# int-brain-lab/mtscomp

Hardware: AMD Instinct MI355X
Metric: compress + decompress GB/s (raw int16) (higher is better)
Workload: dtype int16

## Files before the change

### mtscomp_amd/csrc/inflate.hip

```cpp
#include <stdlib.h>

#include <vector>

#include "common.h"

namespace mts {

struct BitIn {
    const u32 *w;
    u64 nwords;
    u64 widx;
    u64 buf;
    u32 cnt;
    u32 nextw;
    u64 pos;
    u64 end;
    const u32 *lw = nullptr;
    u64 lw0 = 0;
    u32 lwn = 0;
    __device__ __forceinline__ void init(const u8 *base, u64 byte_off, u64 byte_len, u64 start_bit)
    {
        const u64 a = (u64)(base + byte_off);
        w = (const u32 *)(a & ~(u64)3);
        const u64 bit0 = (a & 3) * 8;
// ... 1624 lines not shown
            u32 x = valid ? nt : 0, y = valid ? no : 0;
#pragma unroll
            for (int off = 1; off < 64; off <<= 1) {
                const u32 xx = __shfl_up(x, off, 64), yy = __shfl_up(y, off, 64);
                if (lane >= off) { x += xx; y += yy; }
            }
            __syncthreads();
            if (lane == 63) { s_wt[wave] = x; s_wo[wave] = y; }
            __syncthreads();
            u32 pre_t = 0, pre_o = 0, rt = 0, ro = 0;
#pragma unroll
            for (int w = 0; w < WV_NT / 64; w++) { const u32 a = s_wt[w], bb = s_wo[w]; if (w < wave) { pre_t += a; pre_o += bb; } rt += a; ro += bb; }
            if (nout + ro > limit) emit = false;
            bool bad = false;
            if (valid) {
                u32 *out = tk + ntok + pre_t + (x - nt);
                u64 have = nout + pre_o + (y - no);
                bl.seek(start);
                u32 k = 0;
                while (k < nt) {
                    u32 tok, olen;
                    if (decode_token_lut(bl, L, lutl, lutd, tok, olen) != 0) { bad = true; break; }
                    if ((tok >> 31) && (u64)((tok & 0x7fff) + 1) > have) { bad = true; break; }
                    if (emit) lz_emit_pieces(out + k, tok, olen);
                    k += lz_pieces(tok, olen); have += olen;
                }
            }
            if (tid == 0) s_any = 0;
            __syncthreads();
            if (__any(bad) && lane == 0) s_any = 1;
            if (fstop < WV_NT && tid == fstop) { s_wstop[0] = (u32)fl; s_wstop[1] = ex; }
            if (fstop == WV_NT && tid == WV_NT - 1) s_wstop[1] = ex;
            __syncthreads();
            if (s_any) { st = INF_CORRUPT; break; }
            ntok += emit ? rt : 0; nout += ro;
            if (fstop < WV_NT) {
                if ((int)s_wstop[0] == SPAN_EOB) { done = true; pos = (wb0 << 5) + s_wstop[1]; }
                else st = INF_CORRUPT;
            } else base = (wb0 << 5) + s_wstop[1];
        }
    }
    if (st != INF_OK) r.status = MTS_CHUNK_CORRUPT;
    else {
        const u64 tb = (pos + 7) & ~7ull;
        if (tb + 32 > br.end) r.status = MTS_CHUNK_CORRUPT;
        else {
            const u8 *t = (const u8 *)br.w + (tb >> 3);
            r.adler_stored = ((u32)t[0] << 24) | ((u32)t[1] << 16) | ((u32)t[2] << 8) | t[3];
            r.end_bit = tb + 32;
            if (!emit || nout != limit) r.status = MTS_CHUNK_BADSIZE;
        }
    }
    r.n_out = (u32)(nout < 0xffffffffull ? nout : 0xffffffffull); r.ntok = ntok;
    if (tid == 0) res[ci] = r;
}

constexpr int LZ_THREADS = 1024;
constexpr int LZ_FLUSHERS = 2;
constexpr int LZ_WORKERS = LZ_THREADS / 64 - LZ_FLUSHERS;
constexpr u32 LZ_RING = 65536;
constexpr u32 LZ_REACH = 32768 + 258;
constexpr u32 LZ_FLUSH = 4096;
constexpr u32 LZ_ZLAG = 10;
constexpr u32 LZ_AHEAD = LZ_RING - LZ_ZLAG * LZ_FLUSH;
static_assert(LZ_REACH <= (LZ_ZLAG - 1) * LZ_FLUSH, "a slot must be out of every copy's reach before it is zeroed");
constexpr u32 LZ_BITS_OFF = LZ_RING;
constexpr u32 LZ_CTL_OFF = LZ_RING + LZ_RING / 8 + 16;
constexpr int LZ_LDS = LZ_CTL_OFF + 256;
constexpr u32 LZ_EDGE = LZ_RING - 12;
constexpr u32 LZ_SPIN_MAX = 1u << 20;

#ifndef MTS_LZ_MAXSEG
#define MTS_LZ_MAXSEG 32
#endif
constexpr int LZ_MAXSEG = MTS_LZ_MAXSEG;
constexpr int LZ_STATUS_RETRY = 1000;
constexpr u32 LZ_WIN = 32768;
struct LzPlan {
    u32 nseg;
    u32 g0[LZ_MAXSEG + 1];
    u32 b0[LZ_MAXSEG + 1];
};
constexpr u32 LZ2_CTL_OFF = 2 * LZ_RING + 16;
constexpr int LZ2_LDS = LZ2_CTL_OFF + 256;

constexpr int GS_TILE = 256;

__global__ __launch_bounds__(GS_TILE) void k_inf_gsum(const u32 *__restrict__ tokens, const InfChunk *__restrict__ chunks,
                                                      const InfResult *__restrict__ res, const u64 *__restrict__ gb_off,
                                                      const u64 *__restrict__ tb_off, u32 *__restrict__ gbase,
                                                      u32 *__restrict__ tile_base)
{
    const int ci = blockIdx.y;
    const InfResult r = res[ci];
    if (r.status != MTS_CHUNK_OK) return;
    const u32 ntok = r.ntok, ngroups = (ntok + 63) / 64;
    const u32 g = blockIdx.x * GS_TILE + threadIdx.x;
    if (blockIdx.x * GS_TILE >= ngroups && !(blockIdx.x == 0)) return;
    const u32 *tk = tokens + chunks[ci].tok_off;
    u32 sum = 0;
    {
        const int lane_ = threadIdx.x & 63;
        const u32 g0w = g - (u32)lane_;
        const uint4 *q = (const uint4 *)(tk + (size_t)g0w * 64);
        const u32 nq = ntok > g0w * 64 ? (ntok - g0w * 64) / 4 : 0;
#pragma unroll
        for (int it = 0; it < 16; it++) {
            const u32 i = (u32)it * 64 + (u32)lane_;
            u32 part = 0;
            if (i < nq) {
                const uint4 v = q[i];
                part = ((v.x >> 31) ? ((v.x >> 16) & 0xff) + 3 : 1) + ((v.y >> 31) ? ((v.y >> 16) & 0xff) + 3 : 1) +
                       ((v.z >> 31) ? ((v.z >> 16) & 0xff) + 3 : 1) + ((v.w >> 31) ? ((v.w >> 16) & 0xff) + 3 : 1);
            }
            part += (u32)__builtin_amdgcn_update_dpp(0, (int)part, 0x111, 0xf, 0xf, false);
            part += (u32)__builtin_amdgcn_update_dpp(0, (int)part, 0x112, 0xf, 0xf, false);
            part += (u32)__builtin_amdgcn_update_dpp(0, (int)part, 0x114, 0xf, 0xf, false);
            part += (u32)__builtin_amdgcn_update_dpp(0, (int)part, 0x118, 0xf, 0xf, false);
            const u32 got = (u32)__shfl((int)part, (lane_ & 3) * 16 + 15, 64);
            if ((lane_ >> 2) == it) sum = got;
        }
        if (g < ngroups) {
            const u32 t0 = g * 64, t1 = min(t0 + 64, ntok);
            for (u32 i = max(t0, (g0w * 64 + nq * 4)); i < t1; i++) { const u32 t = tk[i]; sum += (t >> 31) ? ((t >> 16) & 0xff) + 3 : 1; }
        } else sum = 0;
    }
    __shared__ u32 wtot[GS_TILE / 64];
    const int wave = threadIdx.x >> 6, lane = threadIdx.x & 63;
    u32 x = sum;
#pragma unroll
    for (int off = 1; off < 64; off <<= 1) { const u32 y = __shfl_up(x, off, 64); if (lane >= off) x += y; }
    if (lane == 63) wtot[wave] = x;
    __syncthreads();
    u32 add = 0, tot = 0;
    for (int w = 0; w < GS_TILE / 64; w++) { if (w < wave) add += wtot[w]; tot += wtot[w]; }
    if (g < ngroups) gbase[gb_off[ci] + g] = add + x - sum;
    if (threadIdx.x == 0) tile_base[tb_off[ci] + blockIdx.x] = tot;
}

__global__ __launch_bounds__(64) void k_inf_gscan(const InfResult *__restrict__ res, const u64 *__restrict__ tb_off,
                                                  u32 *__restrict__ tile_base)
{
    const int ci = blockIdx.x;
    const InfResult r = res[ci];
    if (r.status != MTS_CHUNK_OK) return;
    const u32 ngroups = (r.ntok + 63) / 64, ntiles = (ngroups + GS_TILE - 1) / GS_TILE;
    u32 *tb = tile_base + tb_off[ci];
    const int lane = threadIdx.x;
    u32 carry = 0;
    for (u32 t0 = 0; t0 < ntiles; t0 += 64) {
        const u32 v = t0 + lane < ntiles ? tb[t0 + lane] : 0;
        u32 x = v;
#pragma unroll
        for (int off = 1; off < 64; off <<= 1) { const u32 y = __shfl_up(x, off, 64); if (lane >= off) x += y; }
        if (t0 + lane < ntiles) tb[t0 + lane] = carry + x - v;
        carry += __shfl(x, 63, 64);
    }
}

__device__ __forceinline__ u32 wave_incl_scan_dpp(u32 x)
{
    x += (u32)__builtin_amdgcn_update_dpp(0, (int)x, 0x111, 0xf, 0xf, false);
    x += (u32)__builtin_amdgcn_update_dpp(0, (int)x, 0x112, 0xf, 0xf, false);
    x += (u32)__builtin_amdgcn_update_dpp(0, (int)x, 0x114, 0xf, 0xf, false);
    x += (u32)__builtin_amdgcn_update_dpp(0, (int)x, 0x118, 0xf, 0xf, false);
    x += (u32)__builtin_amdgcn_update_dpp(0, (int)x, 0x142, 0xa, 0xf, false);
    x += (u32)__builtin_amdgcn_update_dpp(0, (int)x, 0x143, 0xc, 0xf, false);
// ... 205 lines not shown
            }
            const u64 pn = ballot64(pv != 0);
            u64 nx = pn;
            if (pn != pm || (pn & slowm)) idle = 0;
            else if (__builtin_amdgcn_readfirstlane((int)lds_ld(lds_bad))) nx = 0;
            else if (++idle > (1u << 22)) { nx = 0; lds_st(lds_bad, 2); }
            else __builtin_amdgcn_s_sleep(4);
            pm = nx;
        }
        if (prof) { const u64 c3_ = __builtin_readcyclecounter(); pc_wait += c1_ - c0_; pc_pre += c2_ - c1_; pc_loop += c3_ - c2_; pc_groups++; }
    }
    if (prof && lane == 0) {
        u64 *q = prof + ((u64)ci * 16 + wave) * 8;
        q[0] = __builtin_readcyclecounter() - pc_t0; q[1] = pc_wait; q[2] = pc_pre; q[3] = pc_loop; q[4] = pc_iter; q[5] = pc_groups; q[6] = pc_vm; q[7] = pc_sleeps;
    }
    if (lane == 0) lds_st(lds_prog + 4 * wave, 0xffffffffu);
    if (wave == 0) {
        for (u32 waits = 0; flushed() < nout && waits < 4 * LZ_SPIN_MAX; waits++) __builtin_amdgcn_s_sleep(8);
        if (lane == 0 && (lds_ld(lds_bad) || flushed() < nout)) res[ci].status = (pass || lds_ld(lds_bad) == 1) ? MTS_CHUNK_CORRUPT : LZ_STATUS_RETRY;
    }
}

__device__ __forceinline__ void lz2_load_window(u32 data_addr, u32 &x0, u32 &x1, u32 &x2, u32 &x3, u32 &x4)
{
    u32x2 p, q;
    asm volatile("ds_read2_b32 %0, %3 offset1:1\n\tds_read2_b32 %1, %3 offset0:2 offset1:3\n\t"
                 "ds_read_b32 %2, %3 offset:16\n\ts_waitcnt lgkmcnt(0)"
                 : "=&v"(p), "=&v"(q), "=&v"(x4) : "v"(data_addr) : "memory");
    x0 = p.x; x1 = p.y; x2 = q.x; x3 = q.y;
}
__device__ __forceinline__ void lz2_or_window(u32 data_addr, u32 o0, u32 o1, u32 o2, u32 o3, u32 o4)
{
    asm volatile("ds_or_b32 %0, %1\n\tds_or_b32 %0, %2 offset:4\n\tds_or_b32 %0, %3 offset:8\n\tds_or_b32 %0, %4 offset:12\n\t"
                 "ds_or_b32 %0, %5 offset:16"
                 :: "v"(data_addr), "v"(o0), "v"(o1), "v"(o2), "v"(o3), "v"(o4) : "memory");
}
__device__ __forceinline__ void lz2_or_cell(u32 data_addr, u32 w) { asm volatile("ds_or_b32 %0, %1" :: "v"(data_addr), "v"(w) : "memory"); }
__device__ __forceinline__ u32 lz2_load_cell(u32 data_addr)
{
    u32 data;
    asm volatile("ds_read_u16 %0, %1\n\ts_waitcnt lgkmcnt(0)" : "=&v"(data) : "v"(data_addr) : "memory");
    return data;
}
__device__ __forceinline__ u32 lz2_zero_half(u32 y) { return (y - 0x00010001u) & ~y & 0x80008000u; }
__device__ __forceinline__ u32 lz2_pk_min(u32 a, u32 b) { u32 d; asm("v_pk_min_u16 %0, %1, %2" : "=v"(d) : "v"(a), "v"(b)); return d; }

__global__ __launch_bounds__(64) void k_inf_plan(const InfResult *__restrict__ res, const u64 *__restrict__ gb_off,
                                                 const u64 *__restrict__ tb_off, const u32 *__restrict__ gbase,
                                                 const u32 *__restrict__ tile_base, int n_chunks, int nseg_req, LzPlan *__restrict__ plan)
{
    const int ci = blockIdx.x * 64 + threadIdx.x;
    if (ci >= n_chunks) return;
    const InfResult r = res[ci];
    LzPlan *p = plan + ci;
    p->nseg = 1;
    for (int k = 0; k <= LZ_MAXSEG; k++) { p->g0[k] = 0; p->b0[k] = 0; }
    if (r.status == MTS_CHUNK_OK && r.ntok) {
        const u32 ngroups = (r.ntok + 63) / 64;
        const u32 *gbl = gbase + gb_off[ci];
        const u32 *tbs = tile_base + tb_off[ci];
        auto gb = [&](u32 g) -> u32 { return g >= ngroups ? r.n_out : tbs[g / GS_TILE] + gbl[g]; };
        p->g0[1] = ngroups; p->b0[1] = r.n_out;
        for (int ns = nseg_req; ns > 1; ns >>= 1) {
            const u32 per = (ngroups + ns - 1) / ns;
            bool ok = per > 0;
            u32 prev_g = 0, prev_b = 0;
            for (int k = 1; k <= ns && ok; k++) {
                const u32 g = min((u32)k * per, ngroups), b = gb(g);
                if (g <= prev_g) ok = false;
                if (k < ns && b - prev_b < LZ_WIN + 512) ok = false;
                prev_g = g; prev_b = b;
            }
            if (!ok) continue;
            p->nseg = (u32)ns;
            for (int k = 0; k <= ns; k++) { const u32 g = min((u32)k * per, ngroups); p->g0[k] = g; p->b0[k] = gb(g); }
            break;
        }
    }
}
#ifndef MTS_LZ2_STATS
#define MTS_LZ2_STATS 0
#endif
#if MTS_LZ2_STATS
__device__ unsigned long long g_lz2_stats[16];
#define LZ2_CLK() __builtin_readcyclecounter()
#endif
__global__ __launch_bounds__(LZ_THREADS) void k_inf_lz_seg(const u32 *__restrict__ tokens, const InfChunk *__restrict__ chunks,
                                                           InfResult *__restrict__ res, const u64 *__restrict__ gb_off,
                                                           const u64 *__restrict__ tb_off, const u32 *__restrict__ gbase,
                                                           const u32 *__restrict__ tile_base, const LzPlan *__restrict__ plan,
                                                           u16 *__restrict__ sym, int n_workers, int pass, u8 *__restrict__ stream,
                                                           u8 *__restrict__ gflag, u64 *__restrict__ seg_adler)
{
    const int ci = blockIdx.y, seg = blockIdx.x;
    const InfResult r = res[ci];
    if (pass == 2) { if (threadIdx.x == 0 && seg == 0 && r.status == MTS_CHUNK_OK && plan[ci].nseg >= 2) res[ci].status = LZ_STATUS_RETRY; return; }
    if (r.status != (pass ? LZ_STATUS_RETRY : MTS_CHUNK_OK)) return;
    const LzPlan *pl = plan + ci;
    if (pl->nseg < 2 || (u32)seg >= pl->nseg) return;
    const InfChunk ch = chunks[ci];
    extern __shared__ __attribute__((aligned(16))) u8 smem[];
    const u32 lds_data = (u32)(uintptr_t)smem;
    const u32 lds_prog = lds_data + LZ2_CTL_OFF;
    const u32 lds_flnext = lds_prog + 64;
    const u32 lds_bad = lds_prog + 80;
    const int wave = __builtin_amdgcn_readfirstlane((int)(threadIdx.x >> 6)), lane = threadIdx.x & 63;
    const u32 *tk = tokens + ch.tok_off;
    const u32 *gbl = gbase + gb_off[ci];
    const u32 *tbs = tile_base + tb_off[ci];
    u16 *out = sym + ch.stream_off;
    const u32 ntok = r.ntok, ngroups = (ntok + 63) / 64;
    const u32 g_lo = pl->g0[seg], g_hi = pl->g0[seg + 1], B = pl->b0[seg], Bend = pl->b0[seg + 1];
    for (u32 i = threadIdx.x * 16; i < LZ2_CTL_OFF; i += LZ_THREADS * 16) lds_zero16(lds_data + i);
    const u32 q0 = B / LZ_FLUSH;
    if (threadIdx.x < 24) {
        u32 v = 0;
        if (threadIdx.x >= 16 && threadIdx.x < 16 + LZ_FLUSHERS) { const u32 k = threadIdx.x - 16; v = (q0 + ((k - q0) & (LZ_FLUSHERS - 1))) * LZ_FLUSH; }
        lds_st(lds_prog + 4 * threadIdx.x, v);
    }
    __syncthreads();
    if (seg > 0) {
        for (u32 i = threadIdx.x; i < LZ_WIN; i += LZ_THREADS) {
            const u32 ro = (B - LZ_WIN + i) & (LZ_RING - 1);
            lz2_or_cell(lds_data + ((2 * ro) & ~3u), (256 + i + 1) << (16 * (ro & 1)));
        }
    }
    u32 t_n = 0, tb0_n = 0, gl0_n = 0, tb1_n = 0, gl1_n = 0;
    const int LZW = n_workers;
    auto prefetch = [&](u32 h) {
        const u32 h0 = h < g_hi ? h : g_hi - 1, h1 = h + 1 < ngroups ? h + 1 : ngroups - 1;
        const u32 i2 = h0 * 64 + lane;
        t_n = tk[i2 < ntok ? i2 : ntok - 1];
        tb0_n = tbs[h0 / GS_TILE]; gl0_n = gbl[h0]; tb1_n = tbs[h1 / GS_TILE]; gl1_n = gbl[h1];
    };
    if (wave < LZW) {
        prefetch(g_lo + wave);
        if (lane == 0) lds_st(lds_prog + 4 * wave, g_lo + (u32)wave < g_hi ? tb0_n + gl0_n : 0xffffffffu);
    }
    __syncthreads();
    auto safe_bytes = [&]() -> u32 {
        const u32 v = row0_min_dpp(lane < LZW ? lds_ld(lds_prog + 4 * lane) : 0xffffffffu);
        return v < Bend ? v : Bend;
    };
    auto flushed = [&]() -> u32 {
        u32 v = lds_ld(lds_flnext);
#pragma unroll
        for (int k = 1; k < LZ_FLUSHERS; k++) v = min(v, lds_ld(lds_flnext + 4 * k));
        return v;
    };
    if (wave >= LZ_WORKERS) {
        const u32 me = wave - LZ_WORKERS;
        u32 idle = 0;
        u8 *bytes_out = stream + ch.stream_off;
        u8 *gf = gflag + (ch.stream_off >> 12) + ci;
        const u64 nn = ch.n_expect;
        u64 sa = 0, sb = 0;
        for (u32 q = q0 + ((me - q0) & (LZ_FLUSHERS - 1));; q += LZ_FLUSHERS) {
            const u32 lo = q * LZ_FLUSH;
            if (lo >= Bend) break;
            const u32 hi = lo + LZ_FLUSH < Bend ? lo + LZ_FLUSH : Bend;
            while (safe_bytes() < hi) {
                if (++idle > LZ_SPIN_MAX || lds_ld(lds_bad)) { if (lane == 0) { if (!lds_ld(lds_bad)) lds_st(lds_bad, 3); for (int k = 0; k < LZ_FLUSHERS; k++) lds_st(lds_flnext + 4 * k, 0xffffffffu); } return; }
                __builtin_amdgcn_s_sleep(2);
            }
            idle = 0;
            const bool whole = lo >= B && hi == lo + LZ_FLUSH;
            u32x4 c[LZ_FLUSH / 512];
            u32 high = 0;
#pragma unroll
            for (u32 st = 0; st < LZ_FLUSH / 512; st++) {
                const u32 o = lo + st * 512 + lane * 8;
                c[st] = u32x4{0, 0, 0, 0};
                if (o < hi && o + 8 > B) asm volatile("ds_read_b128 %0, %1\n\ts_waitcnt lgkmcnt(0)" : "=v"(c[st]) : "v"(lds_data + 2 * (o & (LZ_RING - 1))) : "memory");
                if (whole || (o >= B && o + 8 <= hi)) { c[st].x -= 0x00010001u; c[st].y -= 0x00010001u; c[st].z -= 0x00010001u; c[st].w -= 0x00010001u; }
                high |= c[st].x | c[st].y | c[st].z | c[st].w;
            }
            if (whole && !any64((high & 0xff00ff00u) != 0)) {
#pragma unroll
                for (u32 st = 0; st < LZ_FLUSH / 512; st++) {
                    const u32 o = lo + st * 512 + lane * 8;
                    const u32 cw[4] = {c[st].x, c[st].y, c[st].z, c[st].w};
                    u32 d[2] = {0, 0}, s1 = 0, s2 = 0;
#pragma unroll
                    for (u32 k = 0; k < 8; k++) {
                        const u32 v = (cw[k >> 1] >> (16 * (k & 1))) & 0xff;
                        d[k >> 2] |= v << (8 * (k & 3));
                        s1 += v; s2 += k * v;
                    }
                    *(uint2 *)(bytes_out + o) = make_uint2(d[0], d[1]);
                    sa += s1; sb += (nn - o) * (u64)s1 - s2;
                }
            } else {
                if (lane == 0) gf[q] = 1;
#pragma unroll
                for (u32 st = 0; st < LZ_FLUSH / 512; st++) {
                    const u32 o = lo + st * 512 + lane * 8;
                    if (o < hi && o + 8 > B) {
                        if (o >= B && o + 8 <= hi) *(u32x4 *)(out + o) = c[st];
                        else { const u32 cw[4] = {c[st].x, c[st].y, c[st].z, c[st].w}; for (u32 k = 0; k < 8; k++) if (o + k >= B && o + k < hi) out[o + k] = (u16)((cw[k >> 1] >> (16 * (k & 1))) - 1u); }
                    }
                }
            }
            if (q >= LZ_ZLAG) {
                const u32 zo = ((q - LZ_ZLAG) * LZ_FLUSH) & (LZ_RING - 1);
#pragma unroll
                for (u32 o = lane * 16; o < 2 * LZ_FLUSH; o += 1024) lds_zero16(lds_data + 2 * zo + o);
            }
            if (lane == 0) lds_st(lds_flnext + 4 * me, lo + LZ_FLUSHERS * LZ_FLUSH);
        }
        for (int d = 32; d; d >>= 1) {
            sa += ((u64)(u32)__shfl_xor((u32)(sa >> 32), d) << 32) | (u32)__shfl_xor((u32)sa, d);
            sb += ((u64)(u32)__shfl_xor((u32)(sb >> 32), d) << 32) | (u32)__shfl_xor((u32)sb, d);
        }
        if (lane == 0) {
            u64 *slot = seg_adler + (((size_t)ci * LZ_MAXSEG + seg) * LZ_FLUSHERS + me) * 2;
            slot[0] = sa % 65521u; slot[1] = sb % 65521u;
            lds_st(lds_flnext + 4 * me, 0xffffffffu);
        }
        return;
    }
    if (wave >= LZW) return;
    u32 fl_seen = 0;
#if MTS_LZ2_STATS
    u64 sg = 0, sit = 0, snm = 0, c_wait = 0, c_pre = 0, c_loop = 0, spend = 0, sslow = 0, sfirst = 0, scp = 0, c_ld = 0;
    const u64 c_start = LZ2_CLK();
#endif
    for (u32 g = g_lo + wave; g < g_hi; g += LZW) {
#if MTS_LZ2_STATS
        const u64 c0_ = LZ2_CLK();
#endif
        const u32 t = t_n, base = tb0_n + gl0_n, next = g + 1 < ngroups ? tb1_n + gl1_n : r.n_out;
        const u32 i = g * 64 + lane;
        const bool act = i < ntok;
        if (lane == 0) lds_st(lds_prog + 4 * wave, base);
        prefetch(g + LZW);
        if (next > LZ_AHEAD) {
            const u32 lim = next - LZ_AHEAD;
            for (u32 waits = 0; fl_seen < lim; waits++) {
                fl_seen = flushed();
                if (fl_seen >= lim) break;
                if (waits > LZ_SPIN_MAX) { if (!lds_ld(lds_bad)) lds_st(lds_bad, 4); break; }
                __builtin_amdgcn_s_sleep(1);
            }
        }
#if MTS_LZ2_STATS
        const u64 c1_ = LZ2_CLK();
#endif
        const bool cp = act && (t >> 31);
        const u32 len = !act ? 0 : cp ? ((t >> 16) & 0xff) + 3 : 1;
        const u32 dst = base + wave_incl_scan_dpp(len) - len;
        const u32 dist = (t & 0x7fff) + 1;
        const u32 src = dst - dist;
        const u32 dofs = dst & (LZ_RING - 1), sofs = src & (LZ_RING - 1);
        u32 pv = cp ? 1u : 0u;
        if (cp && (dist > dst || len > 8)) { pv = 0; lds_st(lds_bad, 1); }
        if (act && !cp) lz2_or_cell(lds_data + ((2 * dofs) & ~3u), ((t & 0xff) + 1u) << (16 * (dofs & 1)));
        const bool slow = sofs > LZ_EDGE || dofs > LZ_EDGE || dist < len;
        const u32 da = lds_data + ((2 * sofs) & ~3u), wa = lds_data + ((2 * dofs) & ~3u);
        const u64 nlo = len >= 4 ? 0ull : ~0ull << (16 * len), nhi = len >= 8 ? 0ull : ~0ull << (16 * max(len, 4u) - 64);
        const u32 n0 = (u32)nlo, n1 = (u32)(nlo >> 32), n2 = (u32)nhi, n3 = (u32)(nhi >> 32);
        const u32 sel = (dofs & 1) ? 0x05040302u : 0x07060504u;
        u32 idle = 0, k = 0, spins = 0;
        const u64 slowm = ballot64(slow);
#if MTS_LZ2_STATS
        const u64 c2_ = LZ2_CLK();
        sg++; scp += __popcll(__ballot(cp)); sslow += __popcll(__ballot(slow && pv));
        bool first_ = true;
#endif
        u64 pm = ballot64(pv != 0);
        while (pm) {
#if MTS_LZ2_STATS
            sit++; spend += __popcll(pm);
#endif
            if (pv != 0 && !slow) {
                u32 x0, x1, x2, x3, x4;
#if MTS_LZ2_STATS
                const u64 cl0_ = LZ2_CLK();
#endif
                lz2_load_window(da, x0, x1, x2, x3, x4);
#if MTS_LZ2_STATS
                c_ld += LZ2_CLK() - cl0_;
#endif
                const u32 ssh = 16 * (sofs & 1);
                const u32 r0 = __builtin_amdgcn_alignbit(x1, x0, ssh), r1 = __builtin_amdgcn_alignbit(x2, x1, ssh);
                const u32 r2 = __builtin_amdgcn_alignbit(x3, x2, ssh), r3 = __builtin_amdgcn_alignbit(x4, x3, ssh);
                const u32 y0 = r0 | n0, y1 = r1 | n1, y2 = r2 | n2, y3 = r3 | n3;
                if (lz2_zero_half(lz2_pk_min(lz2_pk_min(y0, y1), lz2_pk_min(y2, y3))) == 0) {
                    const u32 w0 = y0 ^ n0, w1 = y1 ^ n1, w2 = y2 ^ n2, w3 = y3 ^ n3;
                    lz2_or_window(wa, __builtin_amdgcn_perm(w0, 0u, sel), __builtin_amdgcn_perm(w1, w0, sel), __builtin_amdgcn_perm(w2, w1, sel),
                                  __builtin_amdgcn_perm(w3, w2, sel), __builtin_amdgcn_perm(0u, w3, sel));
                    pv = 0;
                }
            } else if (pv != 0) {
                const u32 so = (src + k) & (LZ_RING - 1), dd = (dst + k) & (LZ_RING - 1);
                const u32 dv = lz2_load_cell(lds_data + 2 * so);
                if (dv) {
                    lz2_or_cell(lds_data + ((2 * dd) & ~3u), dv << (16 * (dd & 1)));
                    if (++k == len) pv = 0;
                    spins = 0;
                } else if ((++spins & 63u) == 0) {
                    if (lds_ld(lds_bad)) pv = 0;
                    else if (spins > (1u << 22)) { pv = 0; lds_st(lds_bad, 2); }
                }
            }
            const u64 pn = ballot64(pv != 0);
#if MTS_LZ2_STATS
            if (first_) { sfirst += __popcll(pm & ~pn); first_ = false; }
            if (pn == pm) snm++;
#endif
            u64 nx = pn;
            if (pn != pm || (pn & slowm)) idle = 0;
            else if (__builtin_amdgcn_readfirstlane((int)lds_ld(lds_bad))) nx = 0;
            else if (++idle > (1u << 22)) { nx = 0; lds_st(lds_bad, 2); }
            else __builtin_amdgcn_s_sleep(4);
            pm = nx;
        }
#if MTS_LZ2_STATS
        { const u64 c3_ = LZ2_CLK(); c_wait += c1_ - c0_; c_pre += c2_ - c1_; c_loop += c3_ - c2_; }
#endif
    }
#if MTS_LZ2_STATS
    if (lane == 0 && pass == 0) {
        const u64 v[13] = {sg, sit, snm, LZ2_CLK() - c_start, c_wait, c_pre, c_loop, spend, sslow, sfirst, scp, 1, c_ld};
        for (int k = 0; k < 13; k++) atomicAdd(&g_lz2_stats[k], v[k]);
    }
#endif
    if (lane == 0) lds_st(lds_prog + 4 * wave, 0xffffffffu);
    if (wave == 0) {
        for (u32 waits = 0; flushed() < Bend && waits < 4 * LZ_SPIN_MAX; waits++) __builtin_amdgcn_s_sleep(8);
        if (lane == 0 && (lds_ld(lds_bad) || flushed() < Bend)) res[ci].status = (pass || lds_ld(lds_bad) == 1) ? MTS_CHUNK_CORRUPT : LZ_STATUS_RETRY;
    }
}

__global__ __launch_bounds__(64) void k_inf_lz_settle(InfResult *__restrict__ res, int n_chunks)
{
    const int ci = blockIdx.x * 64 + threadIdx.x;
    if (ci < n_chunks && res[ci].status == LZ_STATUS_RETRY) res[ci].status = MTS_CHUNK_OK;
}

__global__ __launch_bounds__(1024) void k_inf_windows(const InfChunk *__restrict__ chunks, const InfResult *__restrict__ res,
                                                      const LzPlan *__restrict__ plan, const u16 *__restrict__ sym, u8 *__restrict__ win,
                                                      const u8 *__restrict__ stream, const u8 *__restrict__ gflag)
{
    __shared__ __attribute__((aligned(16))) u8 wl[2][LZ_WIN];
    const int ci = blockIdx.x;
    if (res[ci].status != MTS_CHUNK_OK) return;
    const LzPlan *pl = plan + ci;
    const u32 nseg = pl->nseg;
    if (nseg < 2) return;
    const u16 *cells = sym + chunks[ci].stream_off;
    const u8 *bytes = stream + chunks[ci].stream_off;
    const u8 *gf = gflag + (chunks[ci].stream_off >> 12) + ci;
    u8 *W = win + (size_t)ci * LZ_MAXSEG * LZ_WIN;
    const u32 t = threadIdx.x;
    struct Blk { uint4 c[4]; uint4 b[2]; u32 f; u32 xc; };
    auto fetch = [&](u32 k, Blk &x) {
        const u32 p0 = pl->b0[k] - LZ_WIN;
        const u32 q = ((p0 >> 5) + t) << 5;
        x.f = gf[q / LZ_FLUSH];
#pragma unroll
        for (int j = 0; j < 4; j++) x.c[j] = *(const uint4 *)(cells + q + 8 * j);
        x.b[0] = *(const uint4 *)(bytes + q); x.b[1] = *(const uint4 *)(bytes + q + 16);
        x.xc = 0;
        if (t < (p0 & 31)) { const u32 qx = (p0 & ~31u) + LZ_WIN + t; x.xc = gf[qx / LZ_FLUSH] ? cells[qx] : bytes[qx]; }
    };
    Blk cur, nxt;
    fetch(1, cur);
    for (u32 k = 1; k < nseg; k++) {
        if (k + 1 < nseg) fetch(k + 1, nxt);
        const u32 p0 = pl->b0[k] - LZ_WIN, rot = pl->b0[k - 1];
        const u8 *prev = wl[(k - 1) & 1];
        u8 *mine = wl[k & 1];
        auto tr = [&](u32 c) -> u32 { return c < 256 ? c : (u32)prev[(rot + c - 256) & (LZ_WIN - 1)]; };
        const u32 cw[16] = {cur.c[0].x, cur.c[0].y, cur.c[0].z, cur.c[0].w, cur.c[1].x, cur.c[1].y, cur.c[1].z, cur.c[1].w,
                            cur.c[2].x, cur.c[2].y, cur.c[2].z, cur.c[2].w, cur.c[3].x, cur.c[3].y, cur.c[3].z, cur.c[3].w};
        const u32 bw[8] = {cur.b[0].x, cur.b[0].y, cur.b[0].z, cur.b[0].w, cur.b[1].x, cur.b[1].y, cur.b[1].z, cur.b[1].w};
        u32 ow[8];
#pragma unroll
        for (int j = 0; j < 8; j++) {
            u32 v = bw[j];
            if (cur.f) {
                const u32 a = cw[2 * j], b2 = cw[2 * j + 1];
                v = tr(a & 0xffff) | (tr(a >> 16) << 8) | (tr(b2 & 0xffff) << 16) | (tr(b2 >> 16) << 24);
            }
            ow[j] = v;
        }
        const u32 slot = (((p0 >> 5) + t) << 5) & (LZ_WIN - 1);
        const u32 lowcut = p0 & 31;
        if (t == 0 && lowcut) {
            for (u32 j = lowcut; j < 32; j++) { const u8 v = (u8)(ow[j >> 2] >> (8 * (j & 3))); mine[slot + j] = v; W[(size_t)k * LZ_WIN + slot + j] = v; }
        } else {
            *(uint4 *)(mine + slot) = make_uint4(ow[0], ow[1], ow[2], ow[3]);
            *(uint4 *)(mine + slot + 16) = make_uint4(ow[4], ow[5], ow[6], ow[7]);
            *(uint4 *)(W + (size_t)k * LZ_WIN + slot) = make_uint4(ow[0], ow[1], ow[2], ow[3]);
            *(uint4 *)(W + (size_t)k * LZ_WIN + slot + 16) = make_uint4(ow[4], ow[5], ow[6], ow[7]);
        }
        if (t < lowcut) {
            const u8 v = (u8)tr(cur.xc);
            const u32 sx = ((p0 & ~31u) & (LZ_WIN - 1)) + t;
            mine[sx] = v; W[(size_t)k * LZ_WIN + sx] = v;
        }
        __syncthreads();
        cur = nxt;
    }
}

__global__ __launch_bounds__(256) void k_inf_translate(const InfChunk *__restrict__ chunks, const InfResult *__restrict__ res,
                                                       const LzPlan *__restrict__ plan, const u16 *__restrict__ sym,
                                                       const u8 *__restrict__ win, u8 *__restrict__ stream, u64 *__restrict__ adler_acc,
// ... 255 lines not shown
        hipLaunchKernelGGL(k_inf_passA, dim3(l.total_cand), dim3(64), 0, st, d_cdata, d_chunks, d_fast, (const u32 *)(S + l.slot_chunk),
                           d_cand_pos, d_cand_cnt, d_cres, d_subs, (u32 *)(S + l.rows), (u32 *)(S + l.row_ctr), use_rows ? l.rounds_cap : 0u,
                           (u32 *)(S + l.round_row));
        inflate_mark(engine, st, "inflate_passA");
        hipLaunchKernelGGL(k_inf_chain, dim3(n_chunks), dim3(64), 0, st, d_cdata, d_chunks, d_fast, d_cand_pos, d_cand_cnt, d_cres,
                           d_tblk, d_true_cnt, d_res, d_seq);
        inflate_mark(engine, st, "inflate_chain");
        hipLaunchKernelGGL(k_inf_passB, dim3(l.total_true), dim3(64 * PASSB_WAVES), 0, st, d_cdata, d_chunks, d_fast, (const u32 *)(S + l.tslot_chunk),
                           d_tblk, d_true_cnt, d_cres, d_subs, d_tokens, d_res, use_rows);
        if (use_rows)
            hipLaunchKernelGGL(k_inf_move_rows, dim3(l.total_true), dim3(MOVE_THREADS), 0, st, d_chunks, d_fast, (const u32 *)(S + l.tslot_chunk), d_tblk,
                               d_true_cnt, d_cres, d_subs, (const u32 *)(S + l.rows), (const u32 *)(S + l.round_row), d_tokens);
        inflate_mark(engine, st, "inflate_passB");
    }
    hipLaunchKernelGGL(k_inf_wave, dim3(n_chunks), dim3(WV_NT), 0, st, d_cdata, d_chunks, n_chunks, d_tokens, d_res, fast_path ? d_seq : nullptr);
    inflate_mark(engine, st, "inflate_wave_decoder");
    dbg_status(st, d_res, n_chunks, "after decode");
    {
        u32 max_groups = 1;
        for (int i = 0; i < n_chunks; i++) { const u32 gmax = (u32)(((u64)nn[i] + 2 + 63) / 64); if (gmax > max_groups) max_groups = gmax; }
        dim3 gg((max_groups + GS_TILE - 1) / GS_TILE, n_chunks);
        hipLaunchKernelGGL(k_inf_gsum, gg, dim3(GS_TILE), 0, st, d_tokens, d_chunks, d_res, (const u64 *)(S + l.gb_off),
                           (const u64 *)(S + l.tb_off), (u32 *)(S + l.gbase), (u32 *)(S + l.tile_base));
        hipLaunchKernelGGL(k_inf_gscan, dim3(n_chunks), dim3(64), 0, st, d_res, (const u64 *)(S + l.tb_off), (u32 *)(S + l.tile_base));
        hipLaunchKernelGGL(k_inf_plan, dim3((n_chunks + 63) / 64), dim3(64), 0, st, d_res, (const u64 *)(S + l.gb_off), (const u64 *)(S + l.tb_off),
                           (const u32 *)(S + l.gbase), (const u32 *)(S + l.tile_base), n_chunks, l.nseg, (LzPlan *)(S + l.plan));
    }
    inflate_mark(engine, st, "inflate_offsets");
    u64 *d_prof = nullptr;
    if (getenv("MTS_LZ_PROF")) { MTS_HIP(hipMalloc(&d_prof, (size_t)n_chunks * 16 * 8 * 8)); MTS_HIP(hipMemsetAsync(d_prof, 0, (size_t)n_chunks * 16 * 8 * 8, st)); }
    const int first_pass = getenv("MTS_LZ_FORCE_RETRY") ? 2 : 0;
    hipLaunchKernelGGL(k_inf_lz, dim3(n_chunks), dim3(LZ_THREADS), LZ_LDS, st, d_tokens, d_chunks, d_res, (const u64 *)(S + l.gb_off),
                       (const u64 *)(S + l.tb_off), (const u32 *)(S + l.gbase), (const u32 *)(S + l.tile_base), d_stream, lz_workers,
                       d_prof, (const LzPlan *)(S + l.plan), first_pass);
    hipLaunchKernelGGL(k_inf_lz, dim3(n_chunks), dim3(LZ_THREADS), LZ_LDS, st, d_tokens, d_chunks, d_res, (const u64 *)(S + l.gb_off),
                       (const u64 *)(S + l.tb_off), (const u32 *)(S + l.gbase), (const u32 *)(S + l.tile_base), d_stream, 1,
                       nullptr, (const LzPlan *)(S + l.plan), 1);
    if (l.nseg > 1 && max_n > 0) {
        MTS_HIP(hipMemsetAsync(S + l.gflag, 0, l.seg_adler - l.gflag, st));
        MTS_HIP(hipMemsetAsync(S + l.seg_adler, 0, (size_t)n_chunks * LZ_MAXSEG * LZ_FLUSHERS * 16, st));
        for (int pass = 0; pass < 2; pass++)
            hipLaunchKernelGGL(k_inf_lz_seg, dim3(l.nseg, n_chunks), dim3(LZ_THREADS), LZ2_LDS, st, d_tokens, d_chunks, d_res,
                               (const u64 *)(S + l.gb_off), (const u64 *)(S + l.tb_off), (const u32 *)(S + l.gbase), (const u32 *)(S + l.tile_base),
                               (const LzPlan *)(S + l.plan), (u16 *)(S + l.sym), pass ? 1 : lz_workers, pass ? 1 : first_pass, d_stream,
                               (u8 *)(S + l.gflag), (u64 *)(S + l.seg_adler));
    }
    hipLaunchKernelGGL(k_inf_lz_settle, dim3((n_chunks + 63) / 64), dim3(64), 0, st, d_res, n_chunks);
    MTS_HIP(hipMemsetAsync(d_adler_acc, 0, sizeof(u64) * 2 * n_chunks, st));
    if (l.nseg > 1 && max_n > 0) {
        hipLaunchKernelGGL(k_inf_windows, dim3(n_chunks), dim3(1024), 0, st, d_chunks, d_res, (const LzPlan *)(S + l.plan),
                           (const u16 *)(S + l.sym), (u8 *)(S + l.win), d_stream, (const u8 *)(S + l.gflag));
        hipLaunchKernelGGL(k_inf_translate, dim3((max_n + 16383) / 16384, n_chunks), dim3(256), 0, st, d_chunks, d_res,
                           (const LzPlan *)(S + l.plan), (const u16 *)(S + l.sym), (const u8 *)(S + l.win), d_stream, d_adler_acc, (const u8 *)(S + l.gflag));
    }
    MTS_HIP(hipGetLastError());
    if (d_prof) {
        std::vector<u64> hp((size_t)n_chunks * 16 * 8);
        MTS_HIP(hipStreamSynchronize(st));
        MTS_HIP(hipMemcpy(hp.data(), d_prof, hp.size() * 8, hipMemcpyDeviceToHost));
        MTS_HIP(hipFree(d_prof));
        u64 a[8] = {0, 0, 0, 0, 0, 0, 0, 0}; int nw = 0;
        for (int c = 0; c < n_chunks; c++) for (int w = 0; w < 16; w++) { const u64 *q = &hp[((size_t)c * 16 + w) * 8]; if (!q[5]) continue; nw++; for (int k = 0; k < 8; k++) a[k] += q[k]; }
        if (nw) fprintf(stderr, "[lz prof] waves %d  per wave: total %.0f  wait %.0f  pre %.0f  loop %.0f cycles; groups %.0f  iters/group %.2f  cycles/group %.0f  vmwait %.0f  sleeps %.0f\n", nw,
                        (double)a[0] / nw, (double)a[1] / nw, (double)a[2] / nw, (double)a[3] / nw, (double)a[5] / nw, (double)a[4] / a[5], (double)a[0] / a[5], (double)a[6] / nw, (double)a[7] / nw);
    }
    inflate_mark(engine, st, "inflate_lz");
    dbg_status(st, d_res, n_chunks, "after lz");
    int rc = launch_adler_stream(st, d_stream, (const u64 *)(S + l.so), (const u32 *)(S + l.nn), n_chunks, max_n, d_adler_acc,
                                 (const u32 *)(S + l.plan), (u32)(sizeof(LzPlan) / 4));
    if (rc) return rc;
    hipLaunchKernelGGL(k_inf_finish, dim3((n_chunks + 63) / 64), dim3(64), 0, st, d_chunks, d_res, d_adler_acc, n_chunks,
                       d_status_out, l.nseg > 1 && max_n > 0 ? (const u64 *)(S + l.seg_adler) : nullptr);
    MTS_HIP(hipGetLastError());
    inflate_mark(engine, st, "adler32");
    dbg_status(st, d_res, n_chunks, "after adler");
    return MTS_OK;
}

}

#if MTS_LZ2_STATS
extern "C" int mts_debug_lz2_stats(unsigned long long *out)
{
    if (hipMemcpyFromSymbol(out, HIP_SYMBOL(mts::g_lz2_stats), 128) != hipSuccess) return -1;
    unsigned long long z[16] = {0};
    return hipMemcpyToSymbol(HIP_SYMBOL(mts::g_lz2_stats), z, 128) == hipSuccess ? 0 : -1;
}
#endif
```

Before: 35.44.

## Park stalled LZ back-reference copies on a dedicated helper wave

Sets aside one worker wave in the segmented LZ decode kernel as a parking wave. Worker waves that still have unresolved fast-path back-references after a round write them into per-wave LDS slots and move on to the next group. The parking wave polls those slots and finishes the copies once their source bytes are ready. The goal is to stop a whole worker wave from spinning on a few lanes whose dependencies are not yet resolved. In exchange there is one fewer decoding wave, extra LDS traffic and slot polling, and new progress and termination coordination (done counter, slot-aware progress reporting) that could create stalls.

Measured after the change: 35.01. 0.988x the previous value.

```diff
diff --git a/mtscomp_amd/csrc/inflate.hip b/mtscomp_amd/csrc/inflate.hip
--- a/mtscomp_amd/csrc/inflate.hip
+++ b/mtscomp_amd/csrc/inflate.hip
@@ -1730,7 +1730,18 @@
     u32 b0[LZ_MAXSEG + 1];
 };
 constexpr u32 LZ2_CTL_OFF = 2 * LZ_RING + 16;
-constexpr int LZ2_LDS = LZ2_CTL_OFF + 256;
+#ifndef MTS_LZ2_PARK_ROUNDS
+#define MTS_LZ2_PARK_ROUNDS 1
+#endif
+#ifndef MTS_LZ2_PARK_SLOTS
+#define MTS_LZ2_PARK_SLOTS 4
+#endif
+constexpr int LZ2_PARK_ROUNDS = MTS_LZ2_PARK_ROUNDS;
+constexpr int LZ2_PARK_SLOTS = MTS_LZ2_PARK_SLOTS;
+constexpr int LZ2_WORKERS = LZ2_PARK_ROUNDS ? LZ_WORKERS - 1 : LZ_WORKERS;
+static_assert(LZ2_WORKERS * LZ2_PARK_SLOTS <= 64 && LZ2_PARK_SLOTS <= 16, "one lane of the parking wave per slot; a worker reads its slots in one row");
+constexpr u32 LZ2_PARK_OFF = LZ2_CTL_OFF + 256;
+constexpr int LZ2_LDS = LZ2_PARK_OFF + 64 * 8;
 
 constexpr int GS_TILE = 256;
 
@@ -2102,7 +2113,7 @@
 #define MTS_LZ2_STATS 0
 #endif
 #if MTS_LZ2_STATS
-__device__ unsigned long long g_lz2_stats[16];
+__device__ unsigned long long g_lz2_stats[24];
 #define LZ2_CLK() __builtin_readcyclecounter()
 #endif
 __global__ __launch_bounds__(LZ_THREADS) void k_inf_lz_seg(const u32 *__restrict__ tokens, const InfChunk *__restrict__ chunks,
@@ -2138,6 +2149,7 @@
         if (threadIdx.x >= 16 && threadIdx.x < 16 + LZ_FLUSHERS) { const u32 k = threadIdx.x - 16; v = (q0 + ((k - q0) & (LZ_FLUSHERS - 1))) * LZ_FLUSH; }
         lds_st(lds_prog + 4 * threadIdx.x, v);
     }
+    if (threadIdx.x >= 64 && threadIdx.x < 128) { const u32x2 z = {0, 0}; asm volatile("ds_write_b64 %0, %1" :: "v"(lds_data + LZ2_PARK_OFF + 8 * (threadIdx.x - 64)), "v"(z) : "memory"); }
     __syncthreads();
     if (seg > 0) {
         for (u32 i = threadIdx.x; i < LZ_WIN; i += LZ_THREADS) {
@@ -2146,7 +2158,7 @@
         }
     }
     u32 t_n = 0, tb0_n = 0, gl0_n = 0, tb1_n = 0, gl1_n = 0;
-    const int LZW = n_workers;
+    const int LZW = n_workers < LZ2_WORKERS ? n_workers : LZ2_WORKERS;
     auto prefetch = [&](u32 h) {
         const u32 h0 = h < g_hi ? h : g_hi - 1, h1 = h + 1 < ngroups ? h + 1 : ngroups - 1;
         const u32 i2 = h0 * 64 + lane;
@@ -2239,12 +2251,94 @@
         }
         return;
     }
-    if (wave >= LZW) return;
     u32 fl_seen = 0;
 #if MTS_LZ2_STATS
     u64 sg = 0, sit = 0, snm = 0, c_wait = 0, c_pre = 0, c_loop = 0, spend = 0, sslow = 0, sfirst = 0, scp = 0, c_ld = 0;
+    u64 s_parked = 0, s_adopt = 0, s_drained = 0, s_drit = 0;
     const u64 c_start = LZ2_CLK();
 #endif
+    struct Piece { u32 da, wa, ssh, n0, n1, n2, n3, sel; };
+    auto piece_of = [&](u32 dst_, u32 src_, u32 len_) -> Piece {
+        const u32 dofs_ = dst_ & (LZ_RING - 1), sofs_ = src_ & (LZ_RING - 1);
+        const u64 nlo = len_ >= 4 ? 0ull : ~0ull << (16 * len_), nhi = len_ >= 8 ? 0ull : ~0ull << (16 * max(len_, 4u) - 64);
+        return Piece{lds_data + ((2 * sofs_) & ~3u), lds_data + ((2 * dofs_) & ~3u), 16 * (sofs_ & 1), (u32)nlo, (u32)(nlo >> 32), (u32)nhi,
+                     (u32)(nhi >> 32), (dofs_ & 1) ? 0x05040302u : 0x07060504u};
+    };
+    auto try_piece = [&](const Piece &pc) -> bool {
+        u32 x0, x1, x2, x3, x4;
+#if MTS_LZ2_STATS
+        const u64 cl0_ = LZ2_CLK();
+#endif
+        lz2_load_window(pc.da, x0, x1, x2, x3, x4);
+#if MTS_LZ2_STATS
+        c_ld += LZ2_CLK() - cl0_;
+#endif
+        const u32 r0 = __builtin_amdgcn_alignbit(x1, x0, pc.ssh), r1 = __builtin_amdgcn_alignbit(x2, x1, pc.ssh);
+        const u32 r2 = __builtin_amdgcn_alignbit(x3, x2, pc.ssh), r3 = __builtin_amdgcn_alignbit(x4, x3, pc.ssh);
+        const u32 y0 = r0 | pc.n0, y1 = r1 | pc.n1, y2 = r2 | pc.n2, y3 = r3 | pc.n3;
+        if (lz2_zero_half(lz2_pk_min(lz2_pk_min(y0, y1), lz2_pk_min(y2, y3))) != 0) return false;
+        const u32 w0 = y0 ^ pc.n0, w1 = y1 ^ pc.n1, w2 = y2 ^ pc.n2, w3 = y3 ^ pc.n3;
+        lz2_or_window(pc.wa, __builtin_amdgcn_perm(w0, 0u, pc.sel), __builtin_amdgcn_perm(w1, w0, pc.sel), __builtin_amdgcn_perm(w2, w1, pc.sel),
+                      __builtin_amdgcn_perm(w3, w2, pc.sel), __builtin_amdgcn_perm(0u, w3, pc.sel));
+        return true;
+    };
+    const u32 lds_done = lds_prog + 84;
+    if (LZ2_PARK_ROUNDS && wave == LZ_WORKERS - 1) {
+        const bool mine = lane < LZW * LZ2_PARK_SLOTS;
+        const u32 slot = lds_data + LZ2_PARK_OFF + 8 * lane;
+        u32 pv = 0, idle = 0, empty = 0;
+        Piece pc = piece_of(0, 0, 3);
+        for (;;) {
+            if (mine && pv == 0) {
+                u32x2 e;
+                asm volatile("ds_read_b64 %0, %1\n\ts_waitcnt lgkmcnt(0)" : "=v"(e) : "v"(slot) : "memory");
+                if (e.y) {
+                    pv = 1; empty = 0; pc = piece_of(e.x, e.x - ((e.y & 0x7fff) + 1), e.y >> 16);
+#if MTS_LZ2_STATS
+                    s_adopt++;
+#endif
+                }
+            }
+            const u64 pm = ballot64(pv != 0);
+            if (!pm) {
+                if (__builtin_amdgcn_readfirstlane((int)lds_ld(lds_done)) >= LZW || __builtin_amdgcn_readfirstlane((int)lds_ld(lds_bad))) break;
+                if (++empty > 64 * LZ_SPIN_MAX) { lds_st(lds_bad, 4); break; }
+                __builtin_amdgcn_s_sleep(2);
+                continue;
+            }
+#if MTS_LZ2_STATS
+            s_drit++; s_drained += __popcll(pm);
+#endif
+            if (pv != 0 && try_piece(pc)) { pv = 0; const u32x2 z = {0, 0}; asm volatile("ds_write_b64 %0, %1" :: "v"(slot), "v"(z) : "memory"); }
+            const u64 pn = ballot64(pv != 0);
+            if (pn != pm) idle = 0;
+            else if (__builtin_amdgcn_readfirstlane((int)lds_ld(lds_bad))) break;
+            else if (++idle > (1u << 22)) { lds_st(lds_bad, 2); break; }
+            else __builtin_amdgcn_s_sleep(1);
+        }
+#if MTS_LZ2_STATS
+        if (pass == 0) atomicAdd(&g_lz2_stats[14], s_adopt);
+        if (lane == 0 && pass == 0) {
+            const u64 v[4] = {s_drained, s_drit, 1, LZ2_CLK() - c_start};
+            for (int k = 0; k < 4; k++) atomicAdd(&g_lz2_stats[15 + k], v[k]);
+        }
+#endif
+        return;
+    }
+    if (wave >= LZW) return;
+    const u32 lds_slots = lds_data + LZ2_PARK_OFF + (u32)wave * (8 * LZ2_PARK_SLOTS);
+    u32 occ = 0;
+    auto look = [&](u32 base_) {
+        u32 d = 0xffffffffu, w1 = 0;
+        if (lane < LZ2_PARK_SLOTS) {
+            u32x2 e;
+            asm volatile("ds_read_b64 %0, %1\n\ts_waitcnt lgkmcnt(0)" : "=v"(e) : "v"(lds_slots + 8 * lane) : "memory");
+            w1 = e.y; if (w1) d = e.x;
+        }
+        occ = (u32)ballot64(w1 != 0);
+        const u32 hm = row0_min_dpp(d);
+        if (lane == 0) lds_st(lds_prog + 4 * wave, hm < base_ ? hm : base_);
+    };
     for (u32 g = g_lo + wave; g < g_hi; g += LZW) {
 #if MTS_LZ2_STATS
         const u64 c0_ = LZ2_CLK();
@@ -2252,7 +2346,7 @@
         const u32 t = t_n, base = tb0_n + gl0_n, next = g + 1 < ngroups ? tb1_n + gl1_n : r.n_out;
         const u32 i = g * 64 + lane;
         const bool act = i < ntok;
-        if (lane == 0) lds_st(lds_prog + 4 * wave, base);
+        if (occ) look(base); else if (lane == 0) lds_st(lds_prog + 4 * wave, base);
         prefetch(g + LZW);
         if (next > LZ_AHEAD) {
             const u32 lim = next - LZ_AHEAD;
@@ -2260,6 +2354,7 @@
                 fl_seen = flushed();
                 if (fl_seen >= lim) break;
                 if (waits > LZ_SPIN_MAX) { if (!lds_ld(lds_bad)) lds_st(lds_bad, 4); break; }
+                if (occ) look(base);
                 __builtin_amdgcn_s_sleep(1);
             }
         }
@@ -2276,10 +2371,7 @@
         if (cp && (dist > dst || len > 8)) { pv = 0; lds_st(lds_bad, 1); }
         if (act && !cp) lz2_or_cell(lds_data + ((2 * dofs) & ~3u), ((t & 0xff) + 1u) << (16 * (dofs & 1)));
         const bool slow = sofs > LZ_EDGE || dofs > LZ_EDGE || dist < len;
-        const u32 da = lds_data + ((2 * sofs) & ~3u), wa = lds_data + ((2 * dofs) & ~3u);
-        const u64 nlo = len >= 4 ? 0ull : ~0ull << (16 * len), nhi = len >= 8 ? 0ull : ~0ull << (16 * max(len, 4u) - 64);
-        const u32 n0 = (u32)nlo, n1 = (u32)(nlo >> 32), n2 = (u32)nhi, n3 = (u32)(nhi >> 32);
-        const u32 sel = (dofs & 1) ? 0x05040302u : 0x07060504u;
+        const Piece pc = piece_of(dst, src, len);
         u32 idle = 0, k = 0, spins = 0;
         const u64 slowm = ballot64(slow);
 #if MTS_LZ2_STATS
@@ -2288,29 +2380,13 @@
         bool first_ = true;
 #endif
         u64 pm = ballot64(pv != 0);
+        u32 rounds = 0;
         while (pm) {
 #if MTS_LZ2_STATS
             sit++; spend += __popcll(pm);
 #endif
             if (pv != 0 && !slow) {
-                u32 x0, x1, x2, x3, x4;
-#if MTS_LZ2_STATS
-                const u64 cl0_ = LZ2_CLK();
-#endif
-                lz2_load_window(da, x0, x1, x2, x3, x4);
-#if MTS_LZ2_STATS
-                c_ld += LZ2_CLK() - cl0_;
-#endif
-                const u32 ssh = 16 * (sofs & 1);
-                const u32 r0 = __builtin_amdgcn_alignbit(x1, x0, ssh), r1 = __builtin_amdgcn_alignbit(x2, x1, ssh);
-                const u32 r2 = __builtin_amdgcn_alignbit(x3, x2, ssh), r3 = __builtin_amdgcn_alignbit(x4, x3, ssh);
-                const u32 y0 = r0 | n0, y1 = r1 | n1, y2 = r2 | n2, y3 = r3 | n3;
-                if (lz2_zero_half(lz2_pk_min(lz2_pk_min(y0, y1), lz2_pk_min(y2, y3))) == 0) {
-                    const u32 w0 = y0 ^ n0, w1 = y1 ^ n1, w2 = y2 ^ n2, w3 = y3 ^ n3;
-                    lz2_or_window(wa, __builtin_amdgcn_perm(w0, 0u, sel), __builtin_amdgcn_perm(w1, w0, sel), __builtin_amdgcn_perm(w2, w1, sel),
-                                  __builtin_amdgcn_perm(w3, w2, sel), __builtin_amdgcn_perm(0u, w3, sel));
-                    pv = 0;
-                }
+                if (try_piece(pc)) pv = 0;
             } else if (pv != 0) {
                 const u32 so = (src + k) & (LZ_RING - 1), dd = (dst + k) & (LZ_RING - 1);
                 const u32 dv = lz2_load_cell(lds_data + 2 * so);
@@ -2323,11 +2399,31 @@
                     else if (spins > (1u << 22)) { pv = 0; lds_st(lds_bad, 2); }
                 }
             }
-            const u64 pn = ballot64(pv != 0);
+            u64 pn = ballot64(pv != 0);
 #if MTS_LZ2_STATS
             if (first_) { sfirst += __popcll(pm & ~pn); first_ = false; }
             if (pn == pm) snm++;
 #endif
+            if (LZ2_PARK_ROUNDS && ++rounds == (u32)LZ2_PARK_ROUNDS && (pn & ~slowm)) {
+                const u32 fm = ~occ & ((1u << LZ2_PARK_SLOTS) - 1);
+                if (fm) {
+                    const u64 cand = pn & ~slowm;
+                    const u32 rank = __builtin_amdgcn_mbcnt_hi((u32)(cand >> 32), __builtin_amdgcn_mbcnt_lo((u32)cand, 0u));
+                    u32 sidx = LZ2_PARK_SLOTS, seen = 0;
+#pragma unroll
+                    for (int s_ = 0; s_ < LZ2_PARK_SLOTS; s_++) { if (((fm >> s_) & 1) && seen == rank) sidx = s_; seen += (fm >> s_) & 1; }
+                    if (pv != 0 && !slow && sidx < (u32)LZ2_PARK_SLOTS) {
+                        const u32x2 e = {dst, (dist - 1) | (len << 16)};
+                        asm volatile("ds_write_b64 %0, %1" :: "v"(lds_slots + 8 * sidx), "v"(e) : "memory");
+                        pv = 0;
+                    }
+                    occ = (1u << LZ2_PARK_SLOTS) - 1;
+                    pn = ballot64(pv != 0);
+#if MTS_LZ2_STATS
+                    s_parked += __popcll(cand) - __popcll(pn & ~slowm);
+#endif
+                }
+            }
             u64 nx = pn;
             if (pn != pm || (pn & slowm)) idle = 0;
             else if (__builtin_amdgcn_readfirstlane((int)lds_ld(lds_bad))) nx = 0;
@@ -2339,12 +2435,19 @@
         { const u64 c3_ = LZ2_CLK(); c_wait += c1_ - c0_; c_pre += c2_ - c1_; c_loop += c3_ - c2_; }
 #endif
     }
+    for (u32 waits = 0; occ; waits++) {
+        look(0xffffffffu);
+        if (!occ) break;
+        if (waits > LZ_SPIN_MAX || lds_ld(lds_bad)) { if (!lds_ld(lds_bad)) lds_st(lds_bad, 4); break; }
+        __builtin_amdgcn_s_sleep(1);
+    }
 #if MTS_LZ2_STATS
     if (lane == 0 && pass == 0) {
-        const u64 v[13] = {sg, sit, snm, LZ2_CLK() - c_start, c_wait, c_pre, c_loop, spend, sslow, sfirst, scp, 1, c_ld};
-        for (int k = 0; k < 13; k++) atomicAdd(&g_lz2_stats[k], v[k]);
-    }
-#endif
+        const u64 v[14] = {sg, sit, snm, LZ2_CLK() - c_start, c_wait, c_pre, c_loop, spend, sslow, sfirst, scp, 1, c_ld, s_parked};
+        for (int k = 0; k < 14; k++) atomicAdd(&g_lz2_stats[k], v[k]);
+    }
+#endif
+    if (lane == 0) asm volatile("ds_add_u32 %0, %1" :: "v"(lds_done), "v"(1u) : "memory");
     if (lane == 0) lds_st(lds_prog + 4 * wave, 0xffffffffu);
     if (wave == 0) {
         for (u32 waits = 0; flushed() < Bend && waits < 4 * LZ_SPIN_MAX; waits++) __builtin_amdgcn_s_sleep(8);
@@ -2766,8 +2869,8 @@
 #if MTS_LZ2_STATS
 extern "C" int mts_debug_lz2_stats(unsigned long long *out)
 {
-    if (hipMemcpyFromSymbol(out, HIP_SYMBOL(mts::g_lz2_stats), 128) != hipSuccess) return -1;
-    unsigned long long z[16] = {0};
-    return hipMemcpyToSymbol(HIP_SYMBOL(mts::g_lz2_stats), z, 128) == hipSuccess ? 0 : -1;
-}
-#endif
+    if (hipMemcpyFromSymbol(out, HIP_SYMBOL(mts::g_lz2_stats), 192) != hipSuccess) return -1;
+    unsigned long long z[24] = {0};
+    return hipMemcpyToSymbol(HIP_SYMBOL(mts::g_lz2_stats), z, 192) == hipSuccess ? 0 : -1;
+}
+#endif
```
